# shenyunhang/NA-fWebSOD

Measured on AMD Instinct MI355X. Metric: images/sec (600px, 2000 proposals) VGG16-C5 WSDDN fwd+bwd, higher is better.
Workload: dtype f32 (2xf16 split, 3-pass f16 MFMA, fp32 accumulate)

## Files before the change

include/naws.h:

```cpp
#ifndef NAWS_H_
#define NAWS_H_

#include <stdint.h>

#ifdef __cplusplus
extern "C" {
#endif

#define NAWS_OK 0
#define NAWS_ERR_SHAPE (-1)
#define NAWS_ERR_ARG (-2)
#define NAWS_ERR_NULL (-3)
#define NAWS_ERR_LAUNCH (-4)
#define NAWS_ERR_UNSUPPORTED (-5)

#define NAWS_LAYOUT_NCHW 0
#define NAWS_LAYOUT_NHWC 1

const char* naws_version(void);
int naws_last_hip_error(void);


int naws_conv3x3_c3_nchw_to_nhwc_fwd(const float* X, const float* Wt, const float* bias,
                                     int N, int H, int W, int Cout, int relu,
// ... 199 lines not shown
                                const float* scaleB, float* C, int ldc, int epilogue,
                                const float* bias, float drop_ratio, uint64_t seed, uint32_t* rowmax,
                                int rowmax_seg_cols, uint32_t* colmax, int drop_ld, int drop_col0,
                                void* stream);
int naws_gemm_f32_amax(int transA, int transB, int M, int N, int K, const float* A, int lda,
                       const float* B, int ldb, float* C, int ldc, int batch, int64_t strideA,
                       int64_t strideB, int64_t strideC, int epilogue, const float* bias,
                       int64_t strideBias, const float* aux, int ldaux, float alpha,
                       float drop_ratio, uint64_t seed, int accumulate, uint32_t* rowmax,
                       int rowmax_seg_cols, uint32_t* colmax, const float* colmax_rowmul,
                       void* stream);
int naws_split_f16x2_dual(const float* X, int batch, int rows, int cols, int ld, int64_t strideX,
                          const uint32_t* rowmax, const uint32_t* colmax, const float* rowmul,
                          void* Pn, float* scales_n, int kpad_n, void* Pt, float* scales_t,
                          int kpad_t, void* stream);
int64_t naws_winograd_f16x2_workspace_floats(int N, int H, int W, int Cin, int Cout, int dilation);
int naws_conv3x3_winograd_nhwc_f16x2_fwd(const float* X, const void* U2, const float* scaleU,
                                         const float* bias, int N, int H, int W, int Cin, int Cout,
                                         int dilation, int relu, float* workspace, float* Y,
                                         const uint32_t* amax_in, uint32_t* amax_out, void* stream);
int naws_winograd4_weight_transform(const float* W_oihw, int Cout, int Cin, float* U, void* stream);
int64_t naws_winograd4_f16x2_workspace_floats(int N, int H, int W, int Cin, int Cout, int dilation);
int naws_conv3x3_winograd4_nhwc_f16x2_fwd(const float* X, const void* U2, const float* scaleU,
                                          const float* bias, int N, int H, int W, int Cin, int Cout,
                                          int dilation, int relu, float* workspace, float* Y,
                                          const uint32_t* amax_in, uint32_t* amax_out, void* stream);
int naws_conv3x3_nhwc_f16x2_fwd(const float* X, const void* W2, const float* scaleW,
                                const float* bias, int N, int H, int W, int Cin, int Cout,
                                int dilation, int relu, float* Y, const uint32_t* amax_in,
                                float in_mul, float in_add, uint32_t* amax_out, int amax_out_zeroed,
// ... 128 lines not shown
```

na-fwebsod_amd/csrc/gemm_f32.hip:

```cpp
#include <stdlib.h>
#include <type_traits>
#include "naws_common.h"

namespace {

typedef float f32x16 __attribute__((ext_vector_type(16)));
typedef unsigned int u32x4 __attribute__((ext_vector_type(4)));

struct GemmArgs {
  const float* A;
  const float* B;
  float* C;
  int M, N, K;
  int lda, ldb, ldc;
  long long sA, sB, sC, sBias;
  unsigned bytesA, bytesB;
  const float* bias;
  const float* aux;
  int ldaux;
  float alpha;
  unsigned drop_thr;
  float drop_scale;
  unsigned long long seed;
  int epilogue;
// ... 390 lines not shown
    }
  }
  if (g.am.colmax && col_ok) {
    unsigned* cmx = g.am.colmax + bz * g.am.sCol + col;
    if (cm.x > 0.f) naws_atomic_max_bits(cmx + 0, cm.x);
    if (cm.y > 0.f) naws_atomic_max_bits(cmx + 1, cm.y);
    if (cm.z > 0.f) naws_atomic_max_bits(cmx + 2, cm.z);
    if (cm.w > 0.f) naws_atomic_max_bits(cmx + 3, cm.w);
  }
}

#endif

typedef float sk_f32x4 __attribute__((ext_vector_type(4)));
constexpr int SKM_ROWS = 64;
template <int KS>
__global__ __launch_bounds__(256) void gemm_smallk_mfma_kernel(GemmArgs g) {
  constexpr int KP = KS * 4, LDA_S = KP + 1;
  constexpr bool EARLY = KS <= 10;
  __shared__ float s_rm[SKM_ROWS][4];
  __shared__ float s_cm[1024];
  __shared__ float s_a[SKM_ROWS * LDA_S];
  const long long bz = blockIdx.z;
  const float* A = g.A + bz * g.sA;
  const float* B = g.B + bz * g.sB;
  float* C = g.C + bz * g.sC;
  const float* aux = g.aux ? g.aux + bz * g.sC : nullptr;
  const int lane = threadIdx.x & 63, wave = threadIdx.x >> 6;
  const int l15 = lane & 15, kg = lane >> 4;
  const int m0 = blockIdx.y * SKM_ROWS;
  const int c0 = blockIdx.x * 1024 + wave * 256;
  const bool gate = g.epilogue == NAWS_EPI_GATE_POS;
  for (int i = threadIdx.x; i < SKM_ROWS * KP; i += 256) {
    const int r = i / KP, k = i - r * KP;
    s_a[r * LDA_S + k] = (m0 + r < g.M && k < g.K) ? A[(long long)(m0 + r) * g.lda + k] : 0.f;
  }
  for (int i = threadIdx.x; i < 1024; i += 256) s_cm[i] = 0.f;
  __syncthreads();
  float a[4][KS];
#pragma unroll
  for (int i = 0; i < 4; ++i)
#pragma unroll
    for (int ks = 0; ks < KS; ++ks) a[i][ks] = s_a[(i * 16 + l15) * LDA_S + ks * 4 + kg];
  float cmul[4];
#pragma unroll
  for (int i = 0; i < 4; ++i) {
    const int row = m0 + i * 16 + l15;
    cmul[i] = (g.am.colmul && row < g.M) ? fabsf(g.am.colmul[row]) : 1.f;
  }
  float rmx[4] = {0.f, 0.f, 0.f, 0.f};
  for (int ch = 0; ch < 4; ++ch) {
    const int n0 = c0 + ch * 64;
// ... 10 lines not shown
    auto load_gate = [&](int i) {
      const int row = m0 + i * 16 + l15;
#pragma unroll
      for (int j = 0; j < 4; ++j) {
        const int col = n0 + j * 16 + kg * 4;
        x[i][j] = sk_f32x4{1.f, 1.f, 1.f, 1.f};
        if (gate && row < g.M && col < g.N)
          x[i][j] = *reinterpret_cast<const sk_f32x4*>(aux + (long long)row * g.ldaux + col);
      }
    };
    if constexpr (EARLY) {
#pragma unroll
      for (int i = 0; i < 4; ++i) load_gate(i);
    }
    sk_f32x4 acc[4][4];
#pragma unroll
    for (int i = 0; i < 4; ++i)
#pragma unroll
      for (int j = 0; j < 4; ++j) acc[i][j] = sk_f32x4{0.f, 0.f, 0.f, 0.f};
#pragma unroll
    for (int ks = 0; ks < KS; ++ks)
#pragma unroll
      for (int i = 0; i < 4; ++i)
#pragma unroll
        for (int j = 0; j < 4; ++j)
          acc[i][j] = __builtin_amdgcn_mfma_f32_16x16x4f32(b[j][ks], a[i][ks], acc[i][j], 0, 0, 0);
    float cm[4][4];
#pragma unroll
    for (int j = 0; j < 4; ++j)
#pragma unroll
      for (int e = 0; e < 4; ++e) cm[j][e] = 0.f;
#pragma unroll
    for (int i = 0; i < 4; ++i) {
      const int row = m0 + i * 16 + l15;
      const bool row_on = row < g.M;
      if constexpr (!EARLY) load_gate(i);
      float rm = 0.f;
#pragma unroll
      for (int j = 0; j < 4; ++j) {
        const int col = n0 + j * 16 + kg * 4;
        if (!row_on || col >= g.N) continue;
        sk_f32x4 v = acc[i][j];
        if (gate) {
#pragma unroll
          for (int e = 0; e < 4; ++e) v[e] = x[i][j][e] > 0.f ? v[e] * g.alpha : 0.f;
        }
        sk_f32x4* dst = reinterpret_cast<sk_f32x4*>(C + (long long)row * g.ldc + col);
        if (g.accumulate) {
          const sk_f32x4 o = *dst;
#pragma unroll
          for (int e = 0; e < 4; ++e) v[e] += o[e];
        }
        *dst = v;
#pragma unroll
        for (int e = 0; e < 4; ++e) {
          const float av = fabsf(v[e]);
          rm = fmaxf(rm, av);
          cm[j][e] = fmaxf(cm[j][e], av * cmul[i]);
        }
      }
      rmx[i] = fmaxf(rmx[i], rm);
    }
    if (g.am.colmax) {
#pragma unroll
      for (int j = 0; j < 4; ++j)
#pragma unroll
        for (int e = 0; e < 4; ++e) {
          float v = cm[j][e];
#pragma unroll
          for (int d = 8; d > 0; d >>= 1) v = fmaxf(v, __shfl_xor(v, d));
          if (l15 == 0) s_cm[wave * 256 + ch * 64 + j * 16 + kg * 4 + e] = v;
        }
    }
  }
  if (g.am.rowmax) {
#pragma unroll
    for (int i = 0; i < 4; ++i) {
      float v = rmx[i];
      v = fmaxf(v, __shfl_xor(v, 16));
      v = fmaxf(v, __shfl_xor(v, 32));
      if (kg == 0) s_rm[i * 16 + l15][wave] = v;
    }
  }
  if (g.am.rowmax || g.am.colmax) __syncthreads();
  if (g.am.rowmax && threadIdx.x < SKM_ROWS && m0 + threadIdx.x < g.M) {
    const float m = fmaxf(fmaxf(s_rm[threadIdx.x][0], s_rm[threadIdx.x][1]),
                          fmaxf(s_rm[threadIdx.x][2], s_rm[threadIdx.x][3]));
    unsigned* rowmax = g.am.rowmax + bz * g.am.sRow +
                       (long long)((blockIdx.x * 1024) / g.am.seg_cols) * g.M;
// ... 132 lines not shown
      (!rowmax || g.am.seg_cols % 1024 == 0 || g.am.seg_cols >= N) && gemm_variant() != 7) {
    dim3 grid((unsigned)naws_cdiv(N, 1024), (unsigned)naws_cdiv(M, SKM_ROWS), batch);
#ifdef NAWS_AB
    if (gemm_variant() == 8) grid.y = (unsigned)naws_cdiv(M, SK_ROWS);
#endif
    if (grid.y <= 65535) {
#ifdef NAWS_AB
      if (gemm_variant() == 8) {
        if (K <= 40)
          hipLaunchKernelGGL(gemm_smallk_nn_kernel<40>, grid, dim3(256), 0, s, g);
        else
          hipLaunchKernelGGL(gemm_smallk_nn_kernel<64>, grid, dim3(256), 0, s, g);
      } else
#endif
      if (K <= 40) {
        hipLaunchKernelGGL(gemm_smallk_mfma_kernel<10>, grid, dim3(256), 0, s, g);
      } else {
        hipLaunchKernelGGL(gemm_smallk_mfma_kernel<16>, grid, dim3(256), 0, s, g);
      }
      return naws_check_launch();
    }
  }
  const bool a_kc = !transA, b_kc = transB != 0;
  if (a_kc && b_kc) return dispatch<true, true, false>(g, batch, s);
  if (a_kc && !b_kc) return dispatch<true, false, false>(g, batch, s);
  if (!a_kc && b_kc) return dispatch<false, true, false>(g, batch, s);
  return dispatch<false, false, false>(g, batch, s);
}

extern "C" int64_t naws_gemm_f32_splitk_workspace_floats(int M, int N, int batch, int ksplit) {
  if (M <= 0 || N <= 0 || batch <= 0 || ksplit <= 0) return 0;
  return (int64_t)M * N * batch * ksplit;
}

extern "C" int naws_gemm_f32_splitk(int transA, int transB, int M, int N, int K, const float* A,
                                    int lda, const float* B, int ldb, float* C, int ldc, int batch,
                                    int64_t strideA, int64_t strideB, int64_t strideC, int epilogue,
                                    const float* bias, int64_t strideBias, int ksplit,
                                    float* workspace, void* stream) {
  if (M <= 0 || N <= 0 || K <= 0 || batch <= 0 || ksplit <= 0) return NAWS_ERR_SHAPE;
  NAWS_REQUIRE_PTR(A); NAWS_REQUIRE_PTR(B); NAWS_REQUIRE_PTR(C); NAWS_REQUIRE_PTR(workspace);
  if (epilogue != NAWS_EPI_NONE && epilogue != NAWS_EPI_BIAS) return NAWS_ERR_UNSUPPORTED;
// ... 67 lines not shown
```

na-fwebsod_amd/csrc/gemm_x3.hip:

```cpp
#include "x3_common.h"

#define g_x3_variant naws_knob(NAWS_KNOB_X3)

namespace {

struct XArgs {
  const unsigned short* A;
  const unsigned short* B;
  float* C;
  int M, N, K;
  int ldc;
  long long planeA, planeB;
  long long slabA, slabB;
  long long sA, sB, sC, sBias;
  const float* bias;
  const float* aux;
  int ldaux;
  float alpha;
  unsigned drop_thr;
  float drop_scale;
  unsigned long long seed;
  int epilogue, accumulate;
  int tiles_m, tiles_n, batch;
  int vec4;
// ... 650 lines not shown
      q[1][e] = *reinterpret_cast<const unsigned short*>(&lo);
    }
    const long long dst = ((long long)(k0 / 16 + s) * outer + (o0 + o)) * 16 + hh * 8;
#pragma unroll
    for (int pl = 0; pl < 2; ++pl) {
      u32x4 w;
      w.x = q[pl][0] | ((unsigned)q[pl][1] << 16);
      w.y = q[pl][2] | ((unsigned)q[pl][3] << 16);
      w.z = q[pl][4] | ((unsigned)q[pl][5] << 16);
      w.w = q[pl][6] | ((unsigned)q[pl][7] << 16);
      *reinterpret_cast<u32x4*>(Pb + pl * plane + dst) = w;
    }
  }
}

__device__ __forceinline__ void split2h_pack(const float (&t)[8], float sc, u32x4& hi4, u32x4& lo4) {
  unsigned short q[2][8];
#pragma unroll
  for (int e = 0; e < 8; ++e) {
    const float v = t[e] * sc;
    const _Float16 hi = (_Float16)v;
    float r = v - (float)hi;
    if (!(fabsf(v) <= 65504.f)) r = 0.f;
    const _Float16 lo = (_Float16)r;
    q[0][e] = *reinterpret_cast<const unsigned short*>(&hi);
    q[1][e] = *reinterpret_cast<const unsigned short*>(&lo);
  }
  hi4.x = q[0][0] | ((unsigned)q[0][1] << 16); hi4.y = q[0][2] | ((unsigned)q[0][3] << 16);
  hi4.z = q[0][4] | ((unsigned)q[0][5] << 16); hi4.w = q[0][6] | ((unsigned)q[0][7] << 16);
  lo4.x = q[1][0] | ((unsigned)q[1][1] << 16); lo4.y = q[1][2] | ((unsigned)q[1][3] << 16);
  lo4.z = q[1][4] | ((unsigned)q[1][5] << 16); lo4.w = q[1][6] | ((unsigned)q[1][7] << 16);
}

__global__ __launch_bounds__(256) void split2h_dual_kernel(
    const float* __restrict__ X, int rows, int cols, int ld, long long sx,
    const unsigned* __restrict__ rowmax, const unsigned* __restrict__ colmax,
    const float* __restrict__ rowmul, unsigned short* __restrict__ Pn, float* __restrict__ inv_n,
    int slabs_n, unsigned short* __restrict__ Pt, float* __restrict__ inv_t, int slabs_t, int batch,
    const int* __restrict__ cond, int cond_value, int prows_n) {
  __shared__ float tile[64][65];
  if (cond && *cond != cond_value) return;
  const int bz = blockIdx.z;
  const float* Xb = X + bz * sx;
  const int c0 = blockIdx.x * 64, r0 = blockIdx.y * 64;
  const int tc = threadIdx.x & 63, tr = threadIdx.x >> 6;
#pragma unroll
  for (int i = 0; i < 16; ++i) {
// ... 1 lines not shown
    tile[i * 4 + tr][tc] = (r < rows && c < cols) ? Xb[(long long)r * ld + c] : 0.f;
  }
  __syncthreads();
#pragma unroll
  for (int it = 0; it < 2; ++it) {
    const int u = threadIdx.x + it * 256;
    const int hh = u & 1, o = (u >> 1) & 63, s = u >> 7;
    if (Pn && r0 + o < rows && c0 / 16 + s < slabs_n) {
      float sc, isc;
      f16x2_scales(rowmax[(long long)bz * rows + r0 + o], sc, isc);
      if (c0 == 0 && s == 0 && hh == 0) inv_n[(long long)bz * rows + r0 + o] = isc;
      float t[8];
#pragma unroll
      for (int e = 0; e < 8; ++e) t[e] = tile[o][s * 16 + hh * 8 + e];
      u32x4 hi4, lo4;
      split2h_pack(t, sc, hi4, lo4);
      const long long sp = (long long)slabs_n * 16 * prows_n, plane = (long long)batch * sp;
      const long long dst = bz * sp + ((long long)(c0 / 16 + s) * prows_n + (r0 + o)) * 16 + hh * 8;
      *reinterpret_cast<u32x4*>(Pn + dst) = hi4;
      *reinterpret_cast<u32x4*>(Pn + plane + dst) = lo4;
    }
    if (Pt && c0 + o < cols && r0 / 16 + s < slabs_t) {
      float sc, isc;
      f16x2_scales(colmax[(long long)bz * cols + c0 + o], sc, isc);
      if (r0 == 0 && s == 0 && hh == 0) inv_t[(long long)bz * cols + c0 + o] = isc;
      float t[8];
#pragma unroll
      for (int e = 0; e < 8; ++e) {
        const int kk = s * 16 + hh * 8 + e;
        t[e] = tile[kk][o] * ((rowmul && r0 + kk < rows) ? rowmul[r0 + kk] : 1.f);
      }
      u32x4 hi4, lo4;
      split2h_pack(t, sc, hi4, lo4);
      const long long sp = (long long)slabs_t * 16 * cols, plane = (long long)batch * sp;
      const long long dst = bz * sp + ((long long)(r0 / 16 + s) * cols + (c0 + o)) * 16 + hh * 8;
      *reinterpret_cast<u32x4*>(Pt + dst) = hi4;
      *reinterpret_cast<u32x4*>(Pt + plane + dst) = lo4;
    }
  }
}


__global__ __launch_bounds__(256) void split2h_dual_v4_kernel(
    const float* __restrict__ X, int rows, int cols, int ld, long long sx,
    const unsigned* __restrict__ rowmax, const unsigned* __restrict__ colmax,
    const float* __restrict__ rowmul, unsigned short* __restrict__ Pn, float* __restrict__ inv_n,
    int slabs_n, unsigned short* __restrict__ Pt, float* __restrict__ inv_t, int slabs_t, int batch,
    const int* __restrict__ cond, int cond_value, int prows_n) {
// ... 18 lines not shown
  }
  __syncthreads();
  const int o = tid & 63, s = tid >> 6;
  if (Pn && r0 + o < rows && c0 / 16 + s < slabs_n) {
    float sc, isc;
    f16x2_scales(rowmax[(long long)bz * rows + r0 + o], sc, isc);
    if (c0 == 0 && s == 0) inv_n[(long long)bz * rows + r0 + o] = isc;
    const long long sp = (long long)slabs_n * 16 * prows_n, plane = (long long)batch * sp;
    const long long dst = bz * sp + ((long long)(c0 / 16 + s) * prows_n + (r0 + o)) * 16;
#pragma unroll
    for (int hh = 0; hh < 2; ++hh) {
      const f32x4 a = *reinterpret_cast<const f32x4*>(&tile[o * LDT + s * 16 + hh * 8]);
      const f32x4 b = *reinterpret_cast<const f32x4*>(&tile[o * LDT + s * 16 + hh * 8 + 4]);
      const float t[8] = {a[0], a[1], a[2], a[3], b[0], b[1], b[2], b[3]};
      u32x4 hi4, lo4;
      split2h_pack(t, sc, hi4, lo4);
      *reinterpret_cast<u32x4*>(Pn + dst + hh * 8) = hi4;
      *reinterpret_cast<u32x4*>(Pn + plane + dst + hh * 8) = lo4;
    }
  }
  if (Pt && c0 + o < cols && r0 / 16 + s < slabs_t) {
    float sc, isc;
    f16x2_scales(colmax[(long long)bz * cols + c0 + o], sc, isc);
    if (r0 == 0 && s == 0) inv_t[(long long)bz * cols + c0 + o] = isc;
    const long long sp = (long long)slabs_t * 16 * cols, plane = (long long)batch * sp;
    const long long dst = bz * sp + ((long long)(r0 / 16 + s) * cols + (c0 + o)) * 16;
#pragma unroll
    for (int hh = 0; hh < 2; ++hh) {
      float t[8];
#pragma unroll
      for (int e = 0; e < 8; ++e) {
        const int kk = s * 16 + hh * 8 + e;
        t[e] = tile[kk * LDT + o] * ((rowmul && r0 + kk < rows) ? rowmul[r0 + kk] : 1.f);
      }
      u32x4 hi4, lo4;
      split2h_pack(t, sc, hi4, lo4);
      *reinterpret_cast<u32x4*>(Pt + dst + hh * 8) = hi4;
      *reinterpret_cast<u32x4*>(Pt + plane + dst + hh * 8) = lo4;
    }
  }
}

static void launch_split2h_dual(dim3 grid, hipStream_t s, const float* X, int rows, int cols, int ld,
                                long long sx, const unsigned* rowmax, const unsigned* colmax,
                                const float* rowmul, unsigned short* Pn, float* inv_n, int slabs_n,
                                unsigned short* Pt, float* inv_t, int slabs_t, int batch,
                                const int* cond, int cond_value, int prows_n = 0) {
  if (prows_n <= 0) prows_n = rows;
  const int knob = naws_knob(NAWS_KNOB_SPLIT);
  const bool aligned = (((uintptr_t)X & 15) == 0) && ld % 4 == 0 && cols % 4 == 0 && sx % 4 == 0;
  if (aligned && knob != 1 && (knob == 2 || !Pn))
// ... 453 lines not shown
```

na-fwebsod_amd/csrc/naws_common.h:

```cpp
#pragma once
#include <hip/hip_runtime.h>
#include <stdint.h>
#include <algorithm>
#include "naws.h"

#define NAWS_WAVE 64

extern thread_local int g_naws_last_hip_error;

static inline int naws_check_launch() {
  hipError_t e = hipGetLastError();
  if (e != hipSuccess) {
    g_naws_last_hip_error = (int)e;
    return NAWS_ERR_LAUNCH;
  }
  return NAWS_OK;
}

int naws_allow_lds_impl(const void* kernel, int bytes);
template <typename K>
static inline int naws_allow_lds(K kernel, int bytes = 160 * 1024) {
  return naws_allow_lds_impl(reinterpret_cast<const void*>(kernel), bytes);
}

// ... 34 lines not shown
  return naws_hash_u32(seed, idx) >= thr24;
}
static inline uint32_t naws_drop_threshold(float ratio) {
  double t = (double)ratio * 16777216.0;
  if (t < 0) t = 0;
  if (t > 16777216.0) t = 16777216.0;
  return (uint32_t)t;
}

__device__ __forceinline__ void naws_f16x2_scales(unsigned bound_bits, float& s, float& inv) {
  int e = (int)((bound_bits >> 23) & 0xff);
  if (bound_bits == 0 || e == 0xff) e = 127 + 14;
  e = min(max(e, 40), 250);
  s = __uint_as_float((unsigned)(268 - e) << 23);
  inv = __uint_as_float((unsigned)(e - 14) << 23);
}

__device__ __forceinline__ void sgd_elem(float a, float& m, float& p, float scale, float wd, float LR,
                                         float momentum, int nesterov) {
#pragma clang fp contract(off)
  float t = a * scale;
  t = t + wd * p;
  if (!nesterov) {
    const float adj = LR * t + momentum * m;
    m = adj;
    p = p - adj;
  } else {
    const float mi = m;
    const float mi_new = momentum * mi + LR * t;
    m = mi_new;
// ... 149 lines not shown
```

na-fwebsod_amd/naws_hip/engine.py:

```python

import os

import numpy as np
import torch

from . import lib as L
from . import ops
from .reducer import ArenaReducer, message_plan, message_slice, owner_blocks, owner_pieces

VGG16_CONVS = [
    ('conv1_1', 3, 64, 1), ('conv1_2', 64, 64, 1), ('pool', 2),
    ('conv2_1', 64, 128, 1), ('conv2_2', 128, 128, 1), ('pool', 2),
    ('conv3_1', 128, 256, 1), ('conv3_2', 256, 256, 1), ('conv3_3', 256, 256, 1), ('pool', 2),
    ('conv4_1', 256, 512, 1), ('conv4_2', 512, 512, 1), ('conv4_3', 512, 512, 1), ('pool4',),
    ('conv5_1', 512, 512, None), ('conv5_2', 512, 512, None), ('conv5_3', 512, 512, None),
]

HIDDEN = 4096

_SIDE_STREAMS = {}


def side_stream(device, role):
    key = (str(device), role)
# ... 107 lines not shown
        if any(e % 4 for e in ends):
            raise NotImplementedError('SGD hyper-parameter runs must end on multiples of 4 floats')
        self._seg_host = (list(ends), list(lr_mult), list(wd))
        self.seg_end = torch.tensor(ends, dtype=torch.int64, device=device)
        self.seg_lr_mult = torch.tensor(lr_mult, dtype=torch.float32, device=device)
        self.seg_wd = torch.tensor(wd, dtype=torch.float32, device=device)
        self.lr = torch.zeros((1,), dtype=torch.float32, device=device)
        self._lr_host = 0.0
        self.sgd_iter_count = 0
        self.step_count = 0
        self.conv = {}
        self.stat_state = None
        self.conv_streams = True
        self.fused_planes = True
        self.fuse_wgrad_update = True
        self.defer_update = None
        self.DIRECT_MIN_TILES = 256
        self.WINO_F4_MIN_CIN = 256
        self.X3_DIRECT_MAX_COUT = 256
        self.FC8_KSPLIT = 4
        self.UPDATE_AFTER = 2 if mfma_dtype == 'bf16' else 1
        self.ROI_POOL_ON_CHAINS = True
        self.conv_wino = {}
        self._rm_table = None
        self._fc8_ws = None
        self._w6_updated = None
        self._sgd_regions_rest = None
        self._sgd_regions = None
        self._seg_ring = None
        self._amax5 = None
# ... 635 lines not shown
        gw8 = self.arena.span(G, 'fc8c_w', 'noisy_fc8d_w').view(2, 2 * C, HIDDEN)
        gb8 = self.arena.span(G, 'fc8c_b', 'noisy_fc8d_b')
        ld8 = self.ld8
        pad = ld8 != 2 * C
        dlv = dl.view(rt, 2, ld8).permute(1, 0, 2)
        h7v = h7.view(rt, 2, HIDDEN).permute(1, 0, 2)
        h6v = h6.view(rt, 2, HIDDEN).permute(1, 0, 2)
        bf = self.mfma_dtype == 'bf16'
        x3 = self.mfma_dtype == 'fp32x3'
        h2 = self.mfma_dtype == 'fp16x2'
        red = self.reducer
        w8g = w8
        if pad:
            w8g = self._fc8_operands(w8, self.arena.span(self.params, 'fc8c_b', 'noisy_fc8d_b')
                                     .view(2, 2 * C))[0]
        dz7 = torch.empty_like(h7)
        dz7v = dz7.view(rt, 2, HIDDEN).permute(1, 0, 2)
        dz6 = torch.empty_like(h6)
        dz6v = dz6.view(rt, 2, HIDDEN).permute(1, 0, 2)
        planes_x = h2 and isinstance(x, ops.F16x2)
        if h2:
            sc7n, sc7t, sc6t = self._scales(2, rt), self._scales(2, HIDDEN), self._scales(1, 2 * HIDDEN)
            amax7 = dict(rowmax=ops.amax_words(sc7n), colmax=ops.amax_words(sc7t))
        else:
            amax7 = {}
        ops.gemm(dlv, w8g, False, False, out=dz7v, epilogue=L.EPI_GATE_POS, aux=h7v, alpha=scale,
                 **amax7)
        if h2:
            dz7n, dz7t = ops.split_f16x2_dual(dz7v, sc7n, sc7t)
            ops.gemm_f32_f16x2_nt(dz7n, self._wplanes['w7t'], out=dz6v,
                                  epilogue=L.EPI_GATE_POS, aux=h6v, alpha=scale,
                                  colmax=ops.amax_words(sc6t),
                                  colmax_rowmul=x.inv_scale if planes_x else None)
            del dz7n
        elif x3:
            ops.gemm_f32x3_nt(ops.split_bf16x3(dz7v), self._wplanes['w7t'], out=dz6v,
                              epilogue=L.EPI_GATE_POS, aux=h6v, alpha=scale)
        elif bf:
            ops.gemm_bf16_slab_nt(ops.to_bf16_slab(dz7v), self._wplanes['w7t'], out=dz6v,
                                  epilogue=L.EPI_GATE_POS, aux=h6v, alpha=scale)
        else:
            ops.gemm(dz7v, w7, False, False, out=dz6v, epilogue=L.EPI_GATE_POS, aux=h6v,
                     alpha=scale)
        if h2:
# ... 62 lines not shown
                    self._pipe_enqueue_piece(next_piece)
                next_piece += 1
        if not pipelined:
            ops.colsum(dz6, out=gb6)
        if h2:
            ops.gemm_f32_f16x2_nt(dz7t, self._h6t, out=gw7)
            self._h6t = None
        elif x3:
            ops.gemm_f32x3_nt(ops.split_bf16x3(dz7v, transpose=True),
                              ops.split_bf16x3(h6v, transpose=True), out=gw7)
        elif bf:
            ops.gemm_bf16_slab_nt(ops.to_bf16_slab(dz7v, transpose=True),
                                  ops.to_bf16_slab(h6v, transpose=True), out=gw7)
        else:
            ops.gemm(dz7v, h6v, True, False, out=gw7)
        ops.colsum(dz7, out=gb7)
        if pad:
            gw8p = torch.empty((2, ld8, HIDDEN), device=self.device, dtype=torch.float32)
            self._fc8_gemm(dlv, h7v, True, False, gw8p)
            gw8.copy_(gw8p[:, :2 * C])
            gb8.view(2, 2 * C).copy_(ops.colsum(dl).view(2, ld8)[:, :2 * C])
        else:
            self._fc8_gemm(dlv, h7v, True, False, gw8)
            ops.colsum(dl, out=gb8)
        red.reduce_async(message_slice(self.arena, G, *plan[-1], self.k6))
        if eager:
            self._pipe_state['grads_ready'] = torch.cuda.current_stream(self.device).record_event()
            with torch.cuda.stream(self._upd_stream):
                self._pipe_enqueue_tail()
                self._upd_event = self._upd_stream.record_event()
            self._update_pending, self._update_waiting = True, False
# ... 526 lines not shown
```

na-fwebsod_amd/naws_hip/lib.py:

```python
import ctypes as C
import os

_HERE = os.path.dirname(os.path.abspath(__file__))
LIB_PATH = os.environ.get('NAWS_LIB') or os.path.join(os.path.dirname(_HERE), 'lib',
                                                       'libnaws_hip.so')
_ENV_KNOBS = {'NAWS_GEMM_VARIANT': 'gemm', 'NAWS_X3_VARIANT': 'x3', 'NAWS_H2_VARIANT': 'h2',
              'NAWS_CONV_RING': 'conv_ring', 'NAWS_CONV_BN': 'conv_bn', 'NAWS_ROI_NW': 'roi_nw',
              'NAWS_WINO_VARIANT': 'wino', 'NAWS_SPLIT': 'split', 'NAWS_SGD_WGS': 'sgd_wgs'}

OK, ERR_SHAPE, ERR_ARG, ERR_NULL, ERR_LAUNCH, ERR_UNSUPPORTED = 0, -1, -2, -3, -4, -5
_ERR_NAMES = {
    ERR_SHAPE: 'NAWS_ERR_SHAPE', ERR_ARG: 'NAWS_ERR_ARG', ERR_NULL: 'NAWS_ERR_NULL',
    ERR_LAUNCH: 'NAWS_ERR_LAUNCH', ERR_UNSUPPORTED: 'NAWS_ERR_UNSUPPORTED',
}
LAYOUT_NCHW, LAYOUT_NHWC = 0, 1
EPI_NONE, EPI_BIAS, EPI_BIAS_RELU, EPI_BIAS_RELU_DROP, EPI_GATE_POS = range(5)
UN_LOG, UN_SCALE, UN_REPLACE_NAN, UN_LEAKY_RELU, UN_CLIP, UN_RELU = range(6)
BIN_ADD, BIN_SUB, BIN_MUL, BIN_DIV, BIN_GATE_POS = range(5)
PLANES_F16X2, PLANES_BF16X3, PLANES_BF16 = range(3)

p, i32, i64, u64, f32 = C.c_void_p, C.c_int, C.c_int64, C.c_uint64, C.c_float

PROTOTYPES = {
    'naws_conv3x3_c3_nchw_to_nhwc_fwd': [p, p, p, i32, i32, i32, i32, i32, p, p],
# ... 89 lines not shown
    'naws_emulate_exchange': [p, p, i64, i32, f32, p],
    'naws_gemm_f32_f16x2_nt_xk': [i32, i32, i32, p, i64, i64, p, p, i64, i64, i32, p, p, i32, p],
    'naws_gemm_f32_f16x2_nt_xk_sgd': [i32, i32, i32, p, i64, i64, p, p, i64, i64, i32, p, p, p, i32, p,
                                      f32, f32, f32, i32, i32, i64, p, i64, i32, p, p, p, p, i32, p],
    'naws_conv3x3_winograd_nhwc_f16x2_fwd': [p, p, p, p, i32, i32, i32, i32, i32, i32, i32, p, p, p, p, p],
    'naws_winograd4_weight_transform': [p, i32, i32, p, p],
    'naws_conv3x3_winograd4_nhwc_f16x2_fwd': [p, p, p, p, i32, i32, i32, i32, i32, i32, i32, p, p, p, p, p],
    'naws_gemm_f32_f16x2_nt_amax': [i32, i32, i32, p, i64, i64, p, p, i64, i64, p, p, i32, i32,
                                    i64, i64, i64, i64, i64, i32, p, i64, p, i32, f32, f32, u64, i32,
                                    p, i32, p, p, p],
    'naws_gemm_f32_f16x2_nt_cols': [i32, i32, i32, p, i64, i64, p, p, i64, i64, p, p, i32, i32, p, f32,
                                    u64, p, i32, p, i32, i32, p],
    'naws_gemm_f32_amax': [i32, i32, i32, i32, i32, p, i32, p, i32, p, i32, i32, i64, i64, i64,
                           i32, p, i64, p, i32, f32, f32, u64, i32, p, i32, p, p, p],
    'naws_split_f16x2_dual': [p, i32, i32, i32, i32, i64, p, p, p, p, p, i32, p, p, i32, p],
    'naws_gemm_f32_f16x2_nt': [i32, i32, i32, p, i64, i64, p, p, i64, i64, p, p, i32, i32,
                               i64, i64, i64, i64, i64, i32, p, i64, p, i32, f32, f32, u64, i32, p],
}
SPECIAL = {
    'naws_version': ([], C.c_char_p),
    'naws_last_hip_error': ([], i32),
    'naws_entropy_gate_workspace_floats': ([i32, i32, i32, i32], i64),
    'naws_winograd_workspace_floats': ([i32, i32, i32, i32, i32, i32], i64),
    'naws_nms_workspace_bytes': ([i32, i32], i64),
    'naws_roi_label_workspace_bytes': ([i32, i32, i32], i64),
    'naws_softmax_with_loss_n_workspace_floats': ([i32], i64),
    'naws_roi_pool_workspace_floats': ([i32, i32, i32, i32], i64),
    'naws_winograd_f32x3_workspace_floats': ([i32, i32, i32, i32, i32, i32], i64),
    'naws_winograd_f16x2_workspace_floats': ([i32, i32, i32, i32, i32, i32], i64),
    'naws_winograd4_f16x2_workspace_floats': ([i32, i32, i32, i32, i32, i32], i64),
# ... 60 lines not shown
```

na-fwebsod_amd/naws_hip/ops.py:

```python
import ctypes as C

import numpy as np
import torch

from . import lib as L

_f32 = torch.float32


def _stream():
    return torch.cuda.current_stream().cuda_stream


def _chk(t, name, dtype=_f32):
    if not isinstance(t, torch.Tensor) or not t.is_cuda:
        raise TypeError('%s must be a HIP device tensor (the naws ops have no CPU path)' % name)
    if t.dtype != dtype:
        raise TypeError('%s must be %s, got %s' % (name, dtype, t.dtype))
    if not t.is_contiguous():
        raise ValueError('%s must be contiguous' % name)
    return t


def _ptr(t):
# ... 885 lines not shown
        if o is not None and (tuple(o.planes.shape) != shape or not o.planes.is_contiguous()
                              or o.scales.data_ptr() != sc.data_ptr()):
            raise TypeError('out planes must be contiguous %s with the given scales block' % (shape,))
    for sc, outer in ((scales_n, rows), (scales_t, cols)):
        if sc is not None and (tuple(sc.shape) != (2, *bs, outer) or sc.dtype != _f32
                               or not sc.is_contiguous()):
            raise TypeError('scales must be contiguous fp32 [2, (batch,) outer] blocks')
    if rowmul is not None and (rowmul.numel() != rows or rowmul.dtype != _f32
                               or not rowmul.is_contiguous()):
        raise TypeError('rowmul must be a contiguous fp32 vector with one entry per source row')
    L.call('naws_split_f16x2_dual', x.data_ptr(), batch, rows, cols, x2.stride(0),
           (x.stride(0) if batched else 0), _ptr(scales_n), _ptr(scales_t), _ptr(rowmul),
           _ptr(pn.planes if pn else None), _ptr(scales_n), kn,
           _ptr(pt.planes if pt else None), _ptr(scales_t), kt, _stream())
    return pn, pt


def dropout_mask(seed, ratio, n, device):
    m = torch.empty((n,), device=device, dtype=_f32)
    L.call('naws_dropout_mask', int(seed) & 0xFFFFFFFFFFFFFFFF, float(ratio), n, m.data_ptr(),
           _stream())
    return m


def colsum(x, out=None, accumulate=False):
    assert x.dim() == 2 and x.stride(1) == 1
    m, n = x.shape
    y = out if out is not None else torch.empty((n,), device=x.device, dtype=_f32)
    L.call('naws_colsum_f32', x.data_ptr(), m, n, x.stride(0), y.data_ptr(), int(accumulate),
           _stream())
# ... 402 lines not shown
```

Baseline: 158.8.

## Fuse gated fc7 backward GEMM with f16x2 split and bias column-sum

Replaces the gated small-K GEMM that wrote dz7 to memory, followed by a separate split_f16x2_dual pass and a colsum, with a two-launch scheme. The first pass computes amax and per-block partial column sums without storing C. The second pass recomputes the GEMM, reduces the partials into the bias gradient, and packs hi/lo f16 planes in both layouts directly from registers through shared memory. This removes the dz7 fp32 round trip and the extra kernels, at the cost of doing the cheap small-K MFMA work twice and using a partial-sum workspace.

```diff
diff --git a/include/naws.h b/include/naws.h
--- a/include/naws.h
+++ b/include/naws.h
@@ -237,6 +237,12 @@
                           const uint32_t* rowmax, const uint32_t* colmax, const float* rowmul,
                           void* Pn, float* scales_n, int kpad_n, void* Pt, float* scales_t,
                           int kpad_t, void* stream);
+int naws_gemm_gate_split_f16x2(int M, int N, int K, const float* A, int lda, const float* B,
+                               int ldb, int batch, int64_t strideA, int64_t strideB,
+                               const float* aux, int ldaux, int64_t strideAux, float alpha,
+                               uint32_t* rowmax, uint32_t* colmax, void* Pn, float* scales_n,
+                               int kpad_n, void* Pt, float* scales_t, int kpad_t, float* db,
+                               float* workspace, void* stream);
 int64_t naws_winograd_f16x2_workspace_floats(int N, int H, int W, int Cin, int Cout, int dilation);
 int naws_conv3x3_winograd_nhwc_f16x2_fwd(const float* X, const void* U2, const float* scaleU,
                                          const float* bias, int N, int H, int W, int Cin, int Cout,
diff --git a/na-fwebsod_amd/csrc/gemm_f32.hip b/na-fwebsod_amd/csrc/gemm_f32.hip
--- a/na-fwebsod_amd/csrc/gemm_f32.hip
+++ b/na-fwebsod_amd/csrc/gemm_f32.hip
@@ -428,28 +428,72 @@
 
 typedef float sk_f32x4 __attribute__((ext_vector_type(4)));
 constexpr int SKM_ROWS = 64;
+constexpr int SKP_LD = 68;
+
+struct SkSplitArgs {
+  float* part;
+  unsigned short* Pn;
+  float* inv_n;
+  int slabs_n;
+  unsigned short* Pt;
+  float* inv_t;
+  int slabs_t;
+  float* db;
+  int batch;
+};
+
 template <int KS>
-__global__ __launch_bounds__(256) void gemm_smallk_mfma_kernel(GemmArgs g) {
+__device__ __forceinline__ void smallk_tile_mfma(const float (&a)[4][KS], const float (&b)[4][KS],
+                                                 sk_f32x4 (&acc)[4][4]) {
+#pragma unroll
+  for (int i = 0; i < 4; ++i)
+#pragma unroll
+    for (int j = 0; j < 4; ++j) acc[i][j] = sk_f32x4{0.f, 0.f, 0.f, 0.f};
+#pragma unroll
+  for (int ks = 0; ks < KS; ++ks)
+#pragma unroll
+    for (int i = 0; i < 4; ++i)
+#pragma unroll
+      for (int j = 0; j < 4; ++j)
+        acc[i][j] = __builtin_amdgcn_mfma_f32_16x16x4f32(b[j][ks], a[i][ks], acc[i][j], 0, 0, 0);
+}
+
+template <int KS, int MODE = 0>
+__global__ __launch_bounds__(256) void gemm_smallk_mfma_kernel(GemmArgs g, SkSplitArgs d) {
   constexpr int KP = KS * 4, LDA_S = KP + 1;
   constexpr bool EARLY = KS <= 10;
   __shared__ float s_rm[SKM_ROWS][4];
   __shared__ float s_cm[1024];
   __shared__ float s_a[SKM_ROWS * LDA_S];
+  __shared__ __attribute__((aligned(16))) float s_p[MODE == 2 ? 4 * 16 * SKP_LD : 4];
   const long long bz = blockIdx.z;
   const float* A = g.A + bz * g.sA;
   const float* B = g.B + bz * g.sB;
-  float* C = g.C + bz * g.sC;
+  float* C = MODE == 0 ? g.C + bz * g.sC : nullptr;
   const float* aux = g.aux ? g.aux + bz * g.sC : nullptr;
   const int lane = threadIdx.x & 63, wave = threadIdx.x >> 6;
   const int l15 = lane & 15, kg = lane >> 4;
   const int m0 = blockIdx.y * SKM_ROWS;
   const int c0 = blockIdx.x * 1024 + wave * 256;
   const bool gate = g.epilogue == NAWS_EPI_GATE_POS;
+  if constexpr (MODE == 2) {
+    const long long nt = (long long)gridDim.x * gridDim.y * gridDim.z * 256;
+    for (long long t = (((long long)blockIdx.z * gridDim.y + blockIdx.y) * gridDim.x + blockIdx.x) *
+                           256 + threadIdx.x;
+         t < (long long)d.batch * g.N; t += nt) {
+      const int b = (int)(t / g.N), c = (int)(t - (long long)b * g.N);
+      const float* p = d.part + (long long)b * gridDim.y * g.N + c;
+      float s = 0.f;
+      for (int y = 0; y < (int)gridDim.y; ++y) s += p[(long long)y * g.N];
+      d.db[(long long)b * g.N + c] = s;
+    }
+  }
   for (int i = threadIdx.x; i < SKM_ROWS * KP; i += 256) {
     const int r = i / KP, k = i - r * KP;
     s_a[r * LDA_S + k] = (m0 + r < g.M && k < g.K) ? A[(long long)(m0 + r) * g.lda + k] : 0.f;
   }
-  for (int i = threadIdx.x; i < 1024; i += 256) s_cm[i] = 0.f;
+  if constexpr (MODE != 2)
+    for (int i = threadIdx.x; i < 1024; i += 256) s_cm[i] = 0.f;
   __syncthreads();
   float a[4][KS];
 #pragma unroll
@@ -490,22 +534,75 @@
       for (int i = 0; i < 4; ++i) load_gate(i);
     }
     sk_f32x4 acc[4][4];
-#pragma unroll
-    for (int i = 0; i < 4; ++i)
-#pragma unroll
-      for (int j = 0; j < 4; ++j) acc[i][j] = sk_f32x4{0.f, 0.f, 0.f, 0.f};
-#pragma unroll
-    for (int ks = 0; ks < KS; ++ks)
-#pragma unroll
-      for (int i = 0; i < 4; ++i)
-#pragma unroll
-        for (int j = 0; j < 4; ++j)
-          acc[i][j] = __builtin_amdgcn_mfma_f32_16x16x4f32(b[j][ks], a[i][ks], acc[i][j], 0, 0, 0);
-    float cm[4][4];
+    smallk_tile_mfma<KS>(a, b, acc);
+    if constexpr (MODE == 2) {
+      float* sp = s_p + wave * 16 * SKP_LD;
+      const int pr = l15, ps = kg;
+      const int pc = n0 + lane;
+      float scn, iscn, sct = 1.f, isct = 1.f;
+      if (pc < g.N) naws_f16x2_scales(g.am.colmax[bz * g.am.sCol + pc], sct, isct);
+#pragma unroll
+      for (int i = 0; i < 4; ++i) {
+        const int row = m0 + i * 16 + l15;
+        if constexpr (!EARLY) load_gate(i);
+#pragma unroll
+        for (int j = 0; j < 4; ++j) {
+          const int col = n0 + j * 16 + kg * 4;
+          sk_f32x4 v = acc[i][j];
+          if (gate) {
+#pragma unroll
+            for (int e = 0; e < 4; ++e) v[e] = x[i][j][e] > 0.f ? v[e] * g.alpha : 0.f;
+          }
+          if (row >= g.M || col >= g.N) v = sk_f32x4{0.f, 0.f, 0.f, 0.f};
+          *reinterpret_cast<sk_f32x4*>(sp + l15 * SKP_LD + j * 16 + kg * 4) = v;
+        }
+        __builtin_amdgcn_fence(__ATOMIC_RELEASE, "wavefront");
+        __builtin_amdgcn_wave_barrier();
+        __builtin_amdgcn_fence(__ATOMIC_ACQUIRE, "wavefront");
+        const int prow = m0 + i * 16 + pr;
+        if (prow < g.M && n0 / 16 + ps < d.slabs_n) {
+          naws_f16x2_scales(g.am.rowmax[bz * g.am.sRow + prow], scn, iscn);
+          if (n0 == 0 && ps == 0) d.inv_n[bz * g.M + prow] = iscn;
+          const long long spn = (long long)d.slabs_n * 16 * g.M, plane = (long long)d.batch * spn;
+          const long long dst = bz * spn + ((long long)(n0 / 16 + ps) * g.M + prow) * 16;
+#pragma unroll
+          for (int hh = 0; hh < 2; ++hh) {
+            float t[8];
+#pragma unroll
+            for (int e = 0; e < 8; ++e) t[e] = sp[pr * SKP_LD + ps * 16 + hh * 8 + e];
+            naws_u32x4 hi4, lo4;
+            naws_split2h_pack(t, scn, hi4, lo4);
+            *reinterpret_cast<naws_u32x4*>(d.Pn + dst + hh * 8) = hi4;
+            *reinterpret_cast<naws_u32x4*>(d.Pn + plane + dst + hh * 8) = lo4;
+          }
+        }
+        const int slab = m0 / 16 + i;
+        if (pc < g.N && slab < d.slabs_t) {
+          if (slab == 0) d.inv_t[bz * g.N + pc] = isct;
+          const long long spt = (long long)d.slabs_t * 16 * g.N, plane = (long long)d.batch * spt;
+          const long long dst = bz * spt + ((long long)slab * g.N + pc) * 16;
+#pragma unroll
+          for (int hh = 0; hh < 2; ++hh) {
+            float t[8];
+#pragma unroll
+            for (int e = 0; e < 8; ++e) t[e] = sp[(hh * 8 + e) * SKP_LD + lane];
+            naws_u32x4 hi4, lo4;
+            naws_split2h_pack(t, sct, hi4, lo4);
+            *reinterpret_cast<naws_u32x4*>(d.Pt + dst + hh * 8) = hi4;
+            *reinterpret_cast<naws_u32x4*>(d.Pt + plane + dst + hh * 8) = lo4;
+          }
+        }
+        __builtin_amdgcn_fence(__ATOMIC_RELEASE, "wavefront");
+        __builtin_amdgcn_wave_barrier();
+        __builtin_amdgcn_fence(__ATOMIC_ACQUIRE, "wavefront");
+      }
+      continue;
+    }
+    float cm[4][4], cs[4][4];
 #pragma unroll
     for (int j = 0; j < 4; ++j)
 #pragma unroll
-      for (int e = 0; e < 4; ++e) cm[j][e] = 0.f;
+      for (int e = 0; e < 4; ++e) cm[j][e] = cs[j][e] = 0.f;
 #pragma unroll
     for (int i = 0; i < 4; ++i) {
       const int row = m0 + i * 16 + l15;
@@ -521,13 +618,18 @@
 #pragma unroll
           for (int e = 0; e < 4; ++e) v[e] = x[i][j][e] > 0.f ? v[e] * g.alpha : 0.f;
         }
-        sk_f32x4* dst = reinterpret_cast<sk_f32x4*>(C + (long long)row * g.ldc + col);
-        if (g.accumulate) {
-          const sk_f32x4 o = *dst;
-#pragma unroll
-          for (int e = 0; e < 4; ++e) v[e] += o[e];
-        }
-        *dst = v;
+        if constexpr (MODE == 0) {
+          sk_f32x4* dst = reinterpret_cast<sk_f32x4*>(C + (long long)row * g.ldc + col);
+          if (g.accumulate) {
+            const sk_f32x4 o = *dst;
+#pragma unroll
+            for (int e = 0; e < 4; ++e) v[e] += o[e];
+          }
+          *dst = v;
+        } else {
+#pragma unroll
+          for (int e = 0; e < 4; ++e) cs[j][e] += v[e];
+        }
 #pragma unroll
         for (int e = 0; e < 4; ++e) {
           const float av = fabsf(v[e]);
@@ -537,6 +639,19 @@
       }
       rmx[i] = fmaxf(rmx[i], rm);
     }
+    if constexpr (MODE == 1) {
+      float* prt = d.part + ((long long)bz * gridDim.y + blockIdx.y) * g.N;
+#pragma unroll
+      for (int j = 0; j < 4; ++j)
+#pragma unroll
+        for (int e = 0; e < 4; ++e) {
+          float v = cs[j][e];
+#pragma unroll
+          for (int dd = 1; dd < 16; dd <<= 1) v += __shfl_xor(v, dd);
+          const int col = n0 + j * 16 + kg * 4 + e;
+          if (l15 == 0 && col < g.N) prt[col] = v;
+        }
+    }
     if (g.am.colmax) {
 #pragma unroll
       for (int j = 0; j < 4; ++j)
@@ -544,11 +659,12 @@
         for (int e = 0; e < 4; ++e) {
           float v = cm[j][e];
 #pragma unroll
-          for (int d = 8; d > 0; d >>= 1) v = fmaxf(v, __shfl_xor(v, d));
+          for (int dd = 8; dd > 0; dd >>= 1) v = fmaxf(v, __shfl_xor(v, dd));
           if (l15 == 0) s_cm[wave * 256 + ch * 64 + j * 16 + kg * 4 + e] = v;
         }
     }
   }
+  if constexpr (MODE == 2) return;
   if (g.am.rowmax) {
 #pragma unroll
     for (int i = 0; i < 4; ++i) {
@@ -711,9 +827,9 @@
       } else
 #endif
       if (K <= 40) {
-        hipLaunchKernelGGL(gemm_smallk_mfma_kernel<10>, grid, dim3(256), 0, s, g);
+        hipLaunchKernelGGL(gemm_smallk_mfma_kernel<10>, grid, dim3(256), 0, s, g, SkSplitArgs{});
       } else {
-        hipLaunchKernelGGL(gemm_smallk_mfma_kernel<16>, grid, dim3(256), 0, s, g);
+        hipLaunchKernelGGL(gemm_smallk_mfma_kernel<16>, grid, dim3(256), 0, s, g, SkSplitArgs{});
       }
       return naws_check_launch();
     }
@@ -723,6 +839,46 @@
   if (a_kc && !b_kc) return dispatch<true, false, false>(g, batch, s);
   if (!a_kc && b_kc) return dispatch<false, true, false>(g, batch, s);
   return dispatch<false, false, false>(g, batch, s);
+}
+
+extern "C" int naws_gemm_gate_split_f16x2(int M, int N, int K, const float* A, int lda,
+                                          const float* B, int ldb, int batch, int64_t strideA,
+                                          int64_t strideB, const float* aux, int ldaux,
+                                          int64_t strideAux, float alpha, uint32_t* rowmax,
+                                          uint32_t* colmax, void* Pn, float* scales_n, int kpad_n,
+                                          void* Pt, float* scales_t, int kpad_t, float* db,
+                                          float* workspace, void* stream) {
+  if (M <= 0 || N <= 0 || K <= 0 || batch <= 0) return NAWS_ERR_SHAPE;
+  NAWS_REQUIRE_PTR(A); NAWS_REQUIRE_PTR(B); NAWS_REQUIRE_PTR(aux); NAWS_REQUIRE_PTR(rowmax);
+  NAWS_REQUIRE_PTR(colmax); NAWS_REQUIRE_PTR(Pn); NAWS_REQUIRE_PTR(scales_n); NAWS_REQUIRE_PTR(Pt);
+  NAWS_REQUIRE_PTR(scales_t); NAWS_REQUIRE_PTR(db); NAWS_REQUIRE_PTR(workspace);
+  if (K > SK_MAXK || lda < K || ldb < N || ldaux < N) return NAWS_ERR_SHAPE;
+  if (N % 4 != 0 || ldaux % 4 != 0 || strideAux % 4 != 0 || !ptr16(aux) || !ptr16(Pn) || !ptr16(Pt))
+    return NAWS_ERR_ARG;
+  if (kpad_n != (N + 31) / 32 * 32 || kpad_t != (M + 31) / 32 * 32) return NAWS_ERR_ARG;
+  const long long gy = naws_cdiv(M, SKM_ROWS);
+  if (batch > 65535 || gy > 65535) return NAWS_ERR_UNSUPPORTED;
+  GemmArgs g{};
+  g.A = A; g.B = B; g.M = M; g.N = N; g.K = K; g.lda = lda; g.ldb = ldb;
+  g.sA = strideA; g.sB = strideB; g.sC = strideAux;
+  g.aux = aux; g.ldaux = ldaux; g.alpha = alpha; g.epilogue = NAWS_EPI_GATE_POS;
+  g.am.rowmax = rowmax; g.am.colmax = colmax; g.am.seg_cols = 0x40000000;
+  g.am.sRow = M; g.am.sCol = N;
+  SkSplitArgs d{};
+  d.part = workspace;
+  d.Pn = (unsigned short*)Pn; d.inv_n = scales_n + (long long)batch * M; d.slabs_n = kpad_n / 16;
+  d.Pt = (unsigned short*)Pt; d.inv_t = scales_t + (long long)batch * N; d.slabs_t = kpad_t / 16;
+  d.db = db; d.batch = batch;
+  dim3 grid((unsigned)naws_cdiv(N, 1024), (unsigned)gy, batch);
+  hipStream_t s = (hipStream_t)stream;
+  if (K <= 40) {
+    hipLaunchKernelGGL((gemm_smallk_mfma_kernel<10, 1>), grid, dim3(256), 0, s, g, d);
+    hipLaunchKernelGGL((gemm_smallk_mfma_kernel<10, 2>), grid, dim3(256), 0, s, g, d);
+  } else {
+    hipLaunchKernelGGL((gemm_smallk_mfma_kernel<16, 1>), grid, dim3(256), 0, s, g, d);
+    hipLaunchKernelGGL((gemm_smallk_mfma_kernel<16, 2>), grid, dim3(256), 0, s, g, d);
+  }
+  return naws_check_launch();
 }
 
 extern "C" int64_t naws_gemm_f32_splitk_workspace_floats(int M, int N, int batch, int ksplit) {
diff --git a/na-fwebsod_amd/csrc/gemm_x3.hip b/na-fwebsod_amd/csrc/gemm_x3.hip
--- a/na-fwebsod_amd/csrc/gemm_x3.hip
+++ b/na-fwebsod_amd/csrc/gemm_x3.hip
@@ -688,23 +688,6 @@
   }
 }
 
-__device__ __forceinline__ void split2h_pack(const float (&t)[8], float sc, u32x4& hi4, u32x4& lo4) {
-  unsigned short q[2][8];
-#pragma unroll
-  for (int e = 0; e < 8; ++e) {
-    const float v = t[e] * sc;
-    const _Float16 hi = (_Float16)v;
-    float r = v - (float)hi;
-    if (!(fabsf(v) <= 65504.f)) r = 0.f;
-    const _Float16 lo = (_Float16)r;
-    q[0][e] = *reinterpret_cast<const unsigned short*>(&hi);
-    q[1][e] = *reinterpret_cast<const unsigned short*>(&lo);
-  }
-  hi4.x = q[0][0] | ((unsigned)q[0][1] << 16); hi4.y = q[0][2] | ((unsigned)q[0][3] << 16);
-  hi4.z = q[0][4] | ((unsigned)q[0][5] << 16); hi4.w = q[0][6] | ((unsigned)q[0][7] << 16);
-  lo4.x = q[1][0] | ((unsigned)q[1][1] << 16); lo4.y = q[1][2] | ((unsigned)q[1][3] << 16);
-  lo4.z = q[1][4] | ((unsigned)q[1][5] << 16); lo4.w = q[1][6] | ((unsigned)q[1][7] << 16);
-}
 
 __global__ __launch_bounds__(256) void split2h_dual_kernel(
     const float* __restrict__ X, int rows, int cols, int ld, long long sx,
@@ -736,7 +719,7 @@
 #pragma unroll
       for (int e = 0; e < 8; ++e) t[e] = tile[o][s * 16 + hh * 8 + e];
       u32x4 hi4, lo4;
-      split2h_pack(t, sc, hi4, lo4);
+      naws_split2h_pack(t, sc, hi4, lo4);
       const long long sp = (long long)slabs_n * 16 * prows_n, plane = (long long)batch * sp;
       const long long dst = bz * sp + ((long long)(c0 / 16 + s) * prows_n + (r0 + o)) * 16 + hh * 8;
       *reinterpret_cast<u32x4*>(Pn + dst) = hi4;
@@ -753,7 +736,7 @@
         t[e] = tile[kk][o] * ((rowmul && r0 + kk < rows) ? rowmul[r0 + kk] : 1.f);
       }
       u32x4 hi4, lo4;
-      split2h_pack(t, sc, hi4, lo4);
+      naws_split2h_pack(t, sc, hi4, lo4);
       const long long sp = (long long)slabs_t * 16 * cols, plane = (long long)batch * sp;
       const long long dst = bz * sp + ((long long)(r0 / 16 + s) * cols + (c0 + o)) * 16 + hh * 8;
       *reinterpret_cast<u32x4*>(Pt + dst) = hi4;
@@ -802,7 +785,7 @@
       const f32x4 b = *reinterpret_cast<const f32x4*>(&tile[o * LDT + s * 16 + hh * 8 + 4]);
       const float t[8] = {a[0], a[1], a[2], a[3], b[0], b[1], b[2], b[3]};
       u32x4 hi4, lo4;
-      split2h_pack(t, sc, hi4, lo4);
+      naws_split2h_pack(t, sc, hi4, lo4);
       *reinterpret_cast<u32x4*>(Pn + dst + hh * 8) = hi4;
       *reinterpret_cast<u32x4*>(Pn + plane + dst + hh * 8) = lo4;
     }
@@ -822,7 +805,7 @@
         t[e] = tile[kk * LDT + o] * ((rowmul && r0 + kk < rows) ? rowmul[r0 + kk] : 1.f);
       }
       u32x4 hi4, lo4;
-      split2h_pack(t, sc, hi4, lo4);
+      naws_split2h_pack(t, sc, hi4, lo4);
       *reinterpret_cast<u32x4*>(Pt + dst + hh * 8) = hi4;
       *reinterpret_cast<u32x4*>(Pt + plane + dst + hh * 8) = lo4;
     }
diff --git a/na-fwebsod_amd/csrc/naws_common.h b/na-fwebsod_amd/csrc/naws_common.h
--- a/na-fwebsod_amd/csrc/naws_common.h
+++ b/na-fwebsod_amd/csrc/naws_common.h
@@ -72,6 +72,26 @@
   e = min(max(e, 40), 250);
   s = __uint_as_float((unsigned)(268 - e) << 23);
   inv = __uint_as_float((unsigned)(e - 14) << 23);
+}
+
+typedef unsigned int naws_u32x4 __attribute__((ext_vector_type(4)));
+__device__ __forceinline__ void naws_split2h_pack(const float (&t)[8], float sc, naws_u32x4& hi4,
+                                                  naws_u32x4& lo4) {
+  unsigned short q[2][8];
+#pragma unroll
+  for (int e = 0; e < 8; ++e) {
+    const float v = t[e] * sc;
+    const _Float16 hi = (_Float16)v;
+    float r = v - (float)hi;
+    if (!(fabsf(v) <= 65504.f)) r = 0.f;
+    const _Float16 lo = (_Float16)r;
+    q[0][e] = *reinterpret_cast<const unsigned short*>(&hi);
+    q[1][e] = *reinterpret_cast<const unsigned short*>(&lo);
+  }
+  hi4.x = q[0][0] | ((unsigned)q[0][1] << 16); hi4.y = q[0][2] | ((unsigned)q[0][3] << 16);
+  hi4.z = q[0][4] | ((unsigned)q[0][5] << 16); hi4.w = q[0][6] | ((unsigned)q[0][7] << 16);
+  lo4.x = q[1][0] | ((unsigned)q[1][1] << 16); lo4.y = q[1][2] | ((unsigned)q[1][3] << 16);
+  lo4.z = q[1][4] | ((unsigned)q[1][5] << 16); lo4.w = q[1][6] | ((unsigned)q[1][7] << 16);
 }
 
 __device__ __forceinline__ void sgd_elem(float a, float& m, float& p, float scale, float wd, float LR,
diff --git a/na-fwebsod_amd/naws_hip/engine.py b/na-fwebsod_amd/naws_hip/engine.py
--- a/na-fwebsod_amd/naws_hip/engine.py
+++ b/na-fwebsod_amd/naws_hip/engine.py
@@ -145,6 +145,7 @@
         self.conv_streams = True
         self.fused_planes = True
         self.fuse_wgrad_update = True
+        self.fuse_dz7_split = True
         self.defer_update = None
         self.DIRECT_MIN_TILES = 256
         self.WINO_F4_MIN_CIN = 256
@@ -810,20 +811,25 @@
         if pad:
             w8g = self._fc8_operands(w8, self.arena.span(self.params, 'fc8c_b', 'noisy_fc8d_b')
                                      .view(2, 2 * C))[0]
-        dz7 = torch.empty_like(h7)
-        dz7v = dz7.view(rt, 2, HIDDEN).permute(1, 0, 2)
         dz6 = torch.empty_like(h6)
         dz6v = dz6.view(rt, 2, HIDDEN).permute(1, 0, 2)
         planes_x = h2 and isinstance(x, ops.F16x2)
+        fuse7 = h2 and self.fuse_dz7_split and rt * HIDDEN >= (1 << 20)
         if h2:
             sc7n, sc7t, sc6t = self._scales(2, rt), self._scales(2, HIDDEN), self._scales(1, 2 * HIDDEN)
             amax7 = dict(rowmax=ops.amax_words(sc7n), colmax=ops.amax_words(sc7t))
         else:
             amax7 = {}
-        ops.gemm(dlv, w8g, False, False, out=dz7v, epilogue=L.EPI_GATE_POS, aux=h7v, alpha=scale,
-                 **amax7)
+        if fuse7:
+            dz7n, dz7t = ops.gemm_gate_split_f16x2(dlv, w8g, h7v, scale, sc7n, sc7t, gb7)
+        else:
+            dz7 = torch.empty_like(h7)
+            dz7v = dz7.view(rt, 2, HIDDEN).permute(1, 0, 2)
+            ops.gemm(dlv, w8g, False, False, out=dz7v, epilogue=L.EPI_GATE_POS, aux=h7v,
+                     alpha=scale, **amax7)
+        if h2 and not fuse7:
+            dz7n, dz7t = ops.split_f16x2_dual(dz7v, sc7n, sc7t)
         if h2:
-            dz7n, dz7t = ops.split_f16x2_dual(dz7v, sc7n, sc7t)
             ops.gemm_f32_f16x2_nt(dz7n, self._wplanes['w7t'], out=dz6v,
                                   epilogue=L.EPI_GATE_POS, aux=h6v, alpha=scale,
                                   colmax=ops.amax_words(sc6t),
@@ -916,7 +922,8 @@
                                   ops.to_bf16_slab(h6v, transpose=True), out=gw7)
         else:
             ops.gemm(dz7v, h6v, True, False, out=gw7)
-        ops.colsum(dz7, out=gb7)
+        if not fuse7:
+            ops.colsum(dz7, out=gb7)
         if pad:
             gw8p = torch.empty((2, ld8, HIDDEN), device=self.device, dtype=torch.float32)
             self._fc8_gemm(dlv, h7v, True, False, gw8p)
diff --git a/na-fwebsod_amd/naws_hip/lib.py b/na-fwebsod_amd/naws_hip/lib.py
--- a/na-fwebsod_amd/naws_hip/lib.py
+++ b/na-fwebsod_amd/naws_hip/lib.py
@@ -127,6 +127,8 @@
     'naws_gemm_f32_amax': [i32, i32, i32, i32, i32, p, i32, p, i32, p, i32, i32, i64, i64, i64,
                            i32, p, i64, p, i32, f32, f32, u64, i32, p, i32, p, p, p],
     'naws_split_f16x2_dual': [p, i32, i32, i32, i32, i64, p, p, p, p, p, i32, p, p, i32, p],
+    'naws_gemm_gate_split_f16x2': [i32, i32, i32, p, i32, p, i32, i32, i64, i64, p, i32, i64,
+                                   f32, p, p, p, p, i32, p, p, i32, p, p, p],
     'naws_gemm_f32_f16x2_nt': [i32, i32, i32, p, i64, i64, p, p, i64, i64, p, p, i32, i32,
                                i64, i64, i64, i64, i64, i32, p, i64, p, i32, f32, f32, u64, i32, p],
 }
diff --git a/na-fwebsod_amd/naws_hip/ops.py b/na-fwebsod_amd/naws_hip/ops.py
--- a/na-fwebsod_amd/naws_hip/ops.py
+++ b/na-fwebsod_amd/naws_hip/ops.py
@@ -923,6 +923,33 @@
            _ptr(pn.planes if pn else None), _ptr(scales_n), kn,
            _ptr(pt.planes if pt else None), _ptr(scales_t), kt, _stream())
     return pn, pt
+
+
+def gemm_gate_split_f16x2(a, b, aux, alpha, scales_n, scales_t, db):
+    batch = a.shape[0]
+    a2, b2, x2 = a[0], b[0], aux[0]
+    for t, nm in ((a2, 'A'), (b2, 'B'), (x2, 'aux')):
+        if not t.is_cuda or t.dtype != _f32 or t.stride(-1) != 1:
+            raise TypeError('%s must be a HIP fp32 tensor with a contiguous last dim' % nm)
+    m, k = a2.shape
+    n = b2.shape[1]
+    if b.shape != (batch, k, n) or aux.shape != (batch, m, n):
+        raise L.NawsError('naws_gemm_gate_split_f16x2', L.ERR_SHAPE)
+    for sc, outer in ((scales_n, m), (scales_t, n)):
+        if (tuple(sc.shape) != (2, batch, outer) or sc.dtype != _f32 or not sc.is_contiguous()):
+            raise TypeError('scales must be contiguous fp32 [2, batch, outer] blocks')
+    if tuple(db.shape) not in ((batch, n), (batch * n,)) or db.dtype != _f32 or not db.is_contiguous():
+        raise TypeError('db must be contiguous fp32 [batch, N]')
+    kn, kt = (n + 31) // 32 * 32, (m + 31) // 32 * 32
+    pn = torch.empty((2, batch, kn // 16, m, 16), device=a.device, dtype=torch.float16)
+    pt = torch.empty((2, batch, kt // 16, n, 16), device=a.device, dtype=torch.float16)
+    ws = torch.empty((batch * ((m + 63) // 64) * n,), device=a.device, dtype=_f32)
+    L.call('naws_gemm_gate_split_f16x2', m, n, k, a.data_ptr(), a2.stride(0), b.data_ptr(),
+           b2.stride(0), batch, a.stride(0), b.stride(0), aux.data_ptr(), x2.stride(0),
+           aux.stride(0), float(alpha), amax_words(scales_n).data_ptr(),
+           amax_words(scales_t).data_ptr(), pn.data_ptr(), scales_n.data_ptr(), kn, pt.data_ptr(),
+           scales_t.data_ptr(), kt, db.data_ptr(), ws.data_ptr(), _stream())
+    return F16x2(pn, scales_n), F16x2(pt, scales_t)
 
 
 def dropout_mask(seed, ratio, n, device):
```

Result: no change. 158.7, median of 5 (-0.1%).
